# sinhvt3421/scann--material

Measured on AMD Instinct MI355X. Metric: QM9 molecules/s forward, higher is better.
Workload: dtype f32 (projections: split-fp16 hi/lo operands, 3 v_mfma_f32_32x32x16_f16 per product, fp32 accumulate; everything else fp32)

## Files before the change

### scann--material_amd/csrc/scann_forward.cpp

```cpp
#include "scann_runtime.h"

namespace {

constexpr unsigned kTimingEventFlags = hipEventDisableSystemFence;

int ensure_debug(scann_handle* h, scann_dbatch* db) {
  const int L = h->cfg.n_attention;
  if (db->dbg_layers == L) return SCANN_OK;
  HIPCHK(h, cached_malloc((void**)&db->dbg_c, (size_t)(L + 1) * db->n_atom * D * 4));
  HIPCHK(h, cached_malloc((void**)&db->dbg_ctx, (size_t)std::max(L, 1) * db->n_atom * D * 4));
  if (h->cfg.g_update) HIPCHK(h, cached_malloc((void**)&db->dbg_g, (size_t)(L + 1) * std::max(db->n_edge, 1) * D * 4));
  db->dbg_layers = L;
  return SCANN_OK;
}

int ensure_outputs(scann_handle* h, scann_dbatch* db, const FwdOpts& o) {
  db->out_layers = o.train ? 0 : o.out_layers;
  db->out_flags = o.train ? 0 : o.out_flags;
  db->out_attn = db->out_z = db->out_bf = nullptr;
  if (!db->out_layers && !db->out_flags) return SCANN_OK;
  const scann_config_t& c = h->cfg;
  const size_t n_attn = (size_t)__builtin_popcountll(db->out_layers) * db->n_edge * c.num_head;
  const size_t n_z = db->out_flags & SCANN_OUT_AFTER_LC ? (size_t)db->n_atom * c.global_dim : 0;
  const size_t n_bf = db->out_flags & SCANN_OUT_BF_PROPERTY ? (size_t)db->n_struct * c.dense_out : 0;
// ... 182 lines not shown
  bool on;
  std::vector<hipEvent_t> ev;
  std::vector<int> kind;
  void mark(int k) {
    if (!on) return;
    hipEvent_t e;
    (void)hipEventCreateWithFlags(&e, kTimingEventFlags);
    (void)hipEventRecord(e, s);
    ev.push_back(e);
    kind.push_back(k);
  }
};

int run_forward(scann_handle* h, scann_dbatch* db, hipStream_t s, const FwdOpts& o) {
  scann_handle* const W = o.n_member ? o.members[0] : o.weights ? o.weights : h;
  const FwdTrain* const tr = o.train;
  const McState* const mc = o.mc;
  Timer* const tm = o.tm;
  const bool debug = o.keep_layers < 0 ? h->debug : o.keep_layers != 0;
  const bool exact = o.exact || ((h->force_exact || W->weights_exact) && !debug && !tr);
  const int nm = o.n_member;
  const int64_t wst = o.m_w, ast = o.m_a;
  if (!o.of_set) {
    db->idle = false;
    db->fwd_pending = true;
  }
  if (!W->loaded) return fail(h, SCANN_ERR_WEIGHTS, "forward: weights not loaded");
  const scann_config_t& c = h->cfg;
  const int L = c.n_attention;
  const bool outs = o.out_flags != FWD_OUT_UNTOUCHED;
  const bool fuse_basis = !exact && (h->fuse_basis || mc) && c.g_update && L > 0 && !debug && !tr && db->n_edge > 0;
  if (outs && !tr && o.out_layers && !h->generic && c.g_update && !exact && !fuse_basis && db->n_edge > 0)
    return fail(h, SCANN_ERR_UNSUPPORTED, "forward: local-attention outputs need the fused first layer (not with scann_set_debug or SCANN_FUSE_BASIS=0)");
  HIPCHK(h, wait_upload(db, s));
  if (outs)
    if (const int r = ensure_outputs(h, db, o)) return r;
  const FwdBufs b = o.bufs ? *o.bufs : FwdBufs(db);
  if (h->generic) {
    if (tm) { tm->mark(-1); }
    const int r = run_forward_generic(h, db, s, o, W, b);
    if (tm) tm->mark(3);
    return r;
  }
  if (debug) {
    const int r = ensure_debug(h, db);
    if (r) return r;
  }
  const size_t nA_ = (size_t)db->n_atom * D, nE_ = (size_t)db->n_edge * D;
  auto c_of = [&](int l) { return debug ? db->dbg_c + (size_t)l * nA_ : b.c; };
  auto ctx_of = [&](int l) { return debug ? db->dbg_ctx + (size_t)l * nA_ : b.ctx; };
  auto g_of = [&](int l) { return debug && c.g_update ? db->dbg_g + (size_t)l * nE_ : b.geom; };
  int32_t* const rflag = h->range_flag ? h->range_flag + (o.slot >= 0 ? o.slot : db->last_slot) : nullptr;
  if (tm) tm->mark(-1);
  if (!fuse_basis) {
    if (c.g_update) launch_basis(W->basis, db->dist, db->weight, db->n_edge, g_of(0), s);
    else launch_basis_raw(W->cd, db->dist, db->n_edge, b.gd, s);
  }
  if (tm) tm->mark(0);

  const bool general_embed = c.use_ring || c.feature_cgcnn;
  if (general_embed) {
    for (int m = 0; m < std::max(nm, 1); ++m) {
      EmbedArgs e = nm ? o.members[m]->embed : W->embed;
      e.n_atom = db->n_atom; e.atomic = db->atomic;
      e.c0 = reinterpret_cast<float*>(reinterpret_cast<char*>(b.c0) + m * ast);
      e.ring = c.use_ring ? db->ring : nullptr;
      e.cgcnn = c.feature_cgcnn ? db->cgcnn : nullptr;
      launch_embed(e, s);
    }
    if (tm) tm->mark(0);
  }
  const bool species0 = fuse_basis && h->species_tables && !general_embed && !(mc && mc->p_drop > 0.f) && W->sp_c && db->n_big == 0;
  bool sp_dirty = W->sp_dirty;
  for (int m = 1; m < nm; ++m) sp_dirty |= o.members[m]->sp_dirty;
  if (species0 && sp_dirty) {
    AtomArgs a{};
    a.n_atom = c.n_atoms; a.x = W->lut; a.ffn = 0; a.c = W->sp_c;
    a.range_flag = rflag; a.layer = 0;
    const LayerParams& p = W->layers[0];
    a.mode = 0;
    a.WAh = p.W1h; a.bA = p.bg; a.WBh = p.W3h; a.WCh = p.Wqh; a.bC = p.bq;
    a.oA = W->sp_P1; a.oB = W->sp_P3; a.oC = W->sp_q;
    a.n_member = nm; a.m_w = a.m_x = a.m_o = wst;
    launch_atom(a, s);
    HIPCHK(h, hipStreamSynchronize(s));
    W->sp_dirty = false;
    for (int m = 1; m < nm; ++m) o.members[m]->sp_dirty = false;
  }
  const bool keep_bwd = tr && tr->keep_backward;
  for (int l = 0; l <= L; ++l) {
    const bool keep = keep_bwd && db->keep_K && l < L;
    AtomArgs a{};
    a.n_atom = db->n_atom;
    a.n_member = nm; a.m_w = wst; a.m_x = a.m_o = ast;
    if (l == 0) {
      a.x = general_embed ? b.c0 : W->lut;
      a.x_index = general_embed ? nullptr : db->atomic;
      a.ffn = 0;
      if (!general_embed) a.m_x = wst;
    } else {
      a.x = ctx_of(l - 1);
      a.x_index = nullptr;
      a.ffn = c.use_attn_norm ? 1 : 0;
      const LayerParams& pp = W->layers[l - 1];
      a.Wf1h = pp.Wf1h; a.bf1 = pp.bf1; a.Wf2h = pp.Wf2h; a.bf2 = pp.bf2; a.lnr_g = pp.lnr_g; a.lnr_b = pp.lnr_b;
      if (a.ffn && keep_bwd && db->keep_T2) {
        a.keep_pre1 = db->keep_pre1 + (size_t)(l - 1) * nA_; a.keep_H1 = db->keep_H1 + (size_t)(l - 1) * nA_;
        a.keep_T2 = db->keep_T2 + (size_t)(l - 1) * nA_;
      }
    }
    a.c = c_of(l);
    a.range_flag = rflag; a.layer = l;
    if (tr && tr->drop_p > 0.f) {
      a.drop_p = (l == 0 || c.use_attn_norm) ? tr->drop_p : 0.f;
      a.drop_seed = tr->seed;
      a.drop_tag = l == 0 ? DROP_TAG_EMBED : (unsigned)(l - 1);
    }
    if (mc && mc->p_drop > 0.f && (l == 0 || c.use_attn_norm)) {
      a.drop_p = mc->p_drop;
      a.drop_seed = mc->seed;
      a.drop_tag = l == 0 ? DROP_TAG_EMBED : (unsigned)(l - 1);
      a.mc_rows = mc->rows;
      a.mc_t = mc->t;
    }
    if (l < L) {
      const LayerParams& p = W->layers[l];
      a.mode = c.g_update ? 0 : 1;
      a.WAh = p.W1h; a.bA = p.bg; a.WBh = p.W3h; a.WCh = p.Wqh; a.bC = p.bq;
      a.oA = b.P1; a.oB = b.P3; a.oC = keep ? db->keep_q + (size_t)l * nA_ : b.q;
    } else {
      a.mode = 2;
      a.WAh = W->head.Wah; a.bA = W->head.ba; a.WCh = W->head.Wgqh; a.bC = W->head.bgq; a.WDh = W->head.Wgkh; a.bD = W->head.bgk;
      a.oB = b.gk; a.oC = b.gq;
      if (keep_bwd && db->keep_preA) { a.keep_preA = db->keep_preA; a.keep_z = db->keep_z; }
      a.out_z = outs ? db->out_z : nullptr;
    }
#ifdef SCANN_STAMPS
    if (getenv("SCANN_STAMP_ATOM") && l >= 1 && l < L) {
      const int nt = (db->n_atom + 31) / 32;
      if (!db->stamps) HIPCHK(h, hipMalloc((void**)&db->stamps, (size_t)nt * 16 * sizeof(unsigned long long)));
      a.stamps = db->stamps;
      db->n_stamp = nt;
    }
#endif
    if (exact) {
      a.exact = 1;
      if (l > 0 && a.ffn) {
        const LayerParams& pp = W->layers[l - 1];
        a.Wf1h = reinterpret_cast<const _Float16*>(pp.Wf1p); a.Wf2h = reinterpret_cast<const _Float16*>(pp.Wf2p);
      }
      if (l < L) {
        const LayerParams& p = W->layers[l];
        a.WAh = reinterpret_cast<const _Float16*>(p.W1p); a.WBh = reinterpret_cast<const _Float16*>(p.W3p);
        a.WCh = reinterpret_cast<const _Float16*>(p.Wqp);
      } else {
        a.WAh = reinterpret_cast<const _Float16*>(W->head.Wap); a.WCh = reinterpret_cast<const _Float16*>(W->head.Wgqp);
        a.WDh = reinterpret_cast<const _Float16*>(W->head.Wgkp);
      }
    }
    if (!(species0 && l == 0)) launch_atom(a, s);
    if (tm) tm->mark(l < L ? 1 : 3);
    if (l == L) break;
    EdgeArgs ea{};
    ea.tiles = db->tiles; ea.n_tile = db->n_tile; ea.g_update = c.g_update; ea.tile_rows = db->tile_rows;
    ea.edge_offset = db->edge_offset; ea.edge_col = db->edge_col; ea.edge_row = db->edge_row;
    ea.geom = g_of(l); ea.geom_out = debug && c.g_update ? g_of(l + 1) : nullptr; ea.gd = b.gd; ea.edge_weight = db->weight;
    if (fuse_basis && l == 0) { ea.fuse_basis = 1; ea.dist = db->dist; ea.basis = W->basis; }
    ea.n_edge = db->n_edge;
    ea.geom_rows = fuse_basis ? 0 : 1;
    ea.geom_dead = (l == L - 1 && !debug) ? 1 : 0;
    ea.c = c_of(l); ea.P1 = b.P1; ea.P3 = b.P3; ea.q = keep ? db->keep_q + (size_t)l * nA_ : b.q; ea.ctx = ctx_of(l);
    ea.n_member = nm; ea.m_w = wst; ea.m_a = ea.m_r = ast;
    if (species0 && l == 0) { ea.species = db->atomic; ea.c = W->sp_c; ea.P1 = W->sp_P1; ea.P3 = W->sp_P3; ea.q = W->sp_q; ea.m_r = wst; }
    if (keep) {
      ea.keep_V = db->keep_V + (size_t)l * nE_; ea.keep_K = db->keep_K + (size_t)l * nE_;
      if (db->keep_T) ea.keep_T = db->keep_T + (size_t)l * nE_;
      if (db->keep_ang) ea.keep_ang = db->keep_ang + (size_t)l * nE_;
      db->kept = true;
    }
    ea.p = W->layers[l];
    if (exact) {
      ea.exact = 1;
      ea.p.W2h = reinterpret_cast<const _Float16*>(ea.p.W2p); ea.p.Wkh = reinterpret_cast<const _Float16*>(ea.p.Wkp);
    }
    ea.range_flag = rflag; ea.layer = l;
    const bool sample = !tm && !mc && !o.of_set && h->time_every > 0 && (h->time_count % h->time_every) == 0 && !(fuse_basis && l == 0) &&
                        !(ea.geom_dead && L > 2);
    hipEvent_t ev0 = nullptr, ev1 = nullptr;
    if (sample) {
      (void)hipEventCreateWithFlags(&ev0, kTimingEventFlags);
      (void)hipEventCreateWithFlags(&ev1, kTimingEventFlags);
      (void)hipEventRecord(ev0, s);
    }
    ea.tile_part = db->tile_part; ea.part_buf = b.part_buf;
    ea.xcd_remap = h->xcd_remap;
    ea.attn_out = outs ? attn_out_of(h, db, l) : nullptr;
    if (tr && tr->attn_p > 0.f) {
      ea.attn_drop_p = tr->attn_p;
      ea.attn_drop_seed = tr->seed;
      ea.attn_drop_tag = DROP_TAG_ATTN + (unsigned)l;
    }
    if (mc && mc->p_attn > 0.f && db->n_edge > 0) {
      ea.attn_drop_p = mc->p_attn;
      ea.attn_drop_seed = mc->seed;
      ea.attn_drop_tag = DROP_TAG_ATTN + (unsigned)l;
      ea.mc_rows = mc->rows;
      ea.mc_t = mc->t;
    }
#ifdef SCANN_STAMPS
    if (!getenv("SCANN_STAMP_ATOM") && l == (getenv("SCANN_STAMP_LAYER") ? atoi(getenv("SCANN_STAMP_LAYER")) : L - 1)) {
      if (!db->stamps) HIPCHK(h, hipMalloc((void**)&db->stamps, (size_t)db->n_tile * 16 * sizeof(unsigned long long)));
      ea.stamps = db->stamps;
      db->n_stamp = db->n_tile;
    }
#endif
    launch_edge(ea, s);
    if (nm) launch_edge_merge_set(db->big_tab, db->n_big, b.part_buf, ea.q, ea.p.ln_g, ea.p.ln_b, ea.ctx, rflag, l, nm, ast, wst, s);
    else launch_edge_merge(db->big_tab, db->n_big, b.part_buf, ea.q, ea.p.ln_g, ea.p.ln_b, ea.ctx, rflag, l, s);
    if (ea.attn_out) launch_attn_merge(db->big_tab, db->n_big, b.part_buf, db->edge_offset, db->tile_rows, ea.attn_out, s);
    if (sample) {
      (void)hipEventRecord(ev1, s);
      h->time_ev.push_back(ev0);
      h->time_ev.push_back(ev1);
      h->time_edges.push_back(db->n_edge);
    }
    if (tm) tm->mark(2);
  }
  if (!tm && !mc && !o.of_set) h->time_count++;
  ReadoutArgs r{};
  r.mol_offset = db->mol_offset; r.n_struct = db->n_struct; r.max_atoms = db->max_atoms;
  r.gq = b.gq; r.gk = b.gk; r.use_ga_norm = c.use_ga_norm; r.relu_out = W->cfg.relu_out;
  for (int m = 1; m < nm; ++m) r.relu_out |= o.members[m]->cfg.relu_out << m;
  r.p = W->head; r.ga_attn = b.ga; r.y = b.y; r.bf_out = outs ? db->out_bf : nullptr;
  r.n_member = nm; r.m_w = wst; r.m_a = ast; r.m_g = o.m_g; r.m_y = o.m_y;
  launch_readout(r, s);
  if (tm) tm->mark(3);
  HIPCHK(h, hipGetLastError());
  return SCANN_OK;
}

}

extern "C" {
// ... 226 lines not shown
```

### scann--material_amd/csrc/scann_internal.h

```cpp
#pragma once
#include <hip/hip_runtime.h>
#include <stdint.h>

#include <string>
#include <vector>

namespace scann {

constexpr int D = 128;
constexpr int NHEAD = 8;
constexpr int HDIM = D / NHEAD;
constexpr int NG = 20;
constexpr int LDS_STRIDE = 132;
constexpr int TE_MAX = 64;
constexpr int TA = 64;
constexpr int TQ = 24;
constexpr int WPACK = D * D;
constexpr float WSCALE = 256.f;
constexpr float WMAX = 65504.f / WSCALE;

__host__ __device__ inline float drop_scale(unsigned long long seed, unsigned tag, size_t idx, float p) {
  unsigned long long z = seed + 0x9E3779B97F4A7C15ull * (idx + 1) + ((unsigned long long)tag << 48);
  z = (z ^ (z >> 30)) * 0xBF58476D1CE4E5B9ull;
  z = (z ^ (z >> 27)) * 0x94D049BB133111EBull;
// ... 62 lines not shown
struct EdgeTile {
  int32_t atom_begin, atom_end;
  int32_t edge_begin, edge_end;
};

struct LayerParams {
  const float *bg;
  const float *bq;
  const _Float16 *W1h, *W3h, *Wqh, *Wf1h, *Wf2h;
  const float *bk;
  const _Float16 *W2h, *Wkh;
  const _Float16 *Wfh;
  const float *lng_g, *lng_b;
  const float *ln_g, *ln_b;
  const float *Wfg, *bfg;
  const float *bf1, *bf2, *lnr_g, *lnr_b;
  const float *W1p, *W2p, *W3p, *Wqp, *Wkp, *Wf1p, *Wf2p;
};

struct HeadParams {
  const float *Wap, *ba;
  const float *Wgqp, *bgq, *Wgkp, *bgk;
  const _Float16 *Wah, *Wgqh, *Wgkh;
  const float *Wb, *bb;
  const float *wo, *bo;
};

struct BasisParams {
  const float *Wd, *bd, *Ww, *bw;
  const float *cd, *cw;
  const _Float16 *Wdh, *Wwh;
};


void launch_embed_lut(const float* emb, const float* W, const float* b, int n_species, int emb_dim,
                      float* lut, hipStream_t s);

void launch_basis(const BasisParams& p, const float* dist, const float* weight, int n_edge,
                  float* geom, hipStream_t s);
void launch_basis_raw(const float* cd, const float* dist, int n_edge, float* gd, hipStream_t s);

struct EmbedArgs {
  int32_t n_atom, emb_dim;
  const int32_t* atomic;
  const float* cgcnn;
  const float* ring;
  const float *emb;
  const float *We, *be;
  const float *Wr, *br;
  const float *Wde, *bde;
  float* c0;
};
void launch_embed(const EmbedArgs& a, hipStream_t s);

struct AtomArgs {
  const float* x;
  const int32_t* x_index;
  int32_t n_atom;
  int32_t ffn;
  const _Float16 *Wf1h, *Wf2h;
  const float *bf1, *bf2, *lnr_g, *lnr_b;
  float* c;
  float drop_p;
  uint32_t drop_tag;
  unsigned long long drop_seed;
  int32_t mode;
  const _Float16 *WAh, *WBh, *WCh, *WDh;
  const float *bA;
  const float *bC;
  const float *bD;
  float *oA, *oB, *oC;
  float *keep_pre1, *keep_H1, *keep_T2;
  float *keep_preA, *keep_z;
  unsigned long long* stamps;
  int32_t* range_flag;
  int32_t layer;
  int32_t exact;
  float* out_z;
  const McRow* mc_rows;
  uint32_t mc_t;
  int32_t n_member;
  int64_t m_w, m_x, m_o;
};
void launch_atom(const AtomArgs& a, hipStream_t s);

struct EdgeArgs {
  const EdgeTile* tiles;
  int32_t n_tile;
  int32_t xcd_remap;
  const int32_t* tile_part;
  float* part_buf;
  int32_t g_update;
  const int32_t* edge_offset;
  const int32_t* edge_col;
  const int32_t* edge_row;
  float* geom;
  float *keep_V, *keep_T, *keep_ang, *keep_K;
  float* geom_out;
  int32_t tile_rows;
  int32_t n_edge;
  int32_t geom_rows;
  int32_t geom_dead;
  const float* gd;
  const float* edge_weight;
  int32_t fuse_basis;
  const int32_t* species;
  const float* dist;
  BasisParams basis;
  const float *c, *P1, *P3, *q;
  float* ctx;
  float attn_drop_p;
  uint32_t attn_drop_tag;
  unsigned long long attn_drop_seed;
  unsigned long long* stamps;
  int32_t* range_flag;
  int32_t layer;
  int32_t exact;
  LayerParams p;
  float* attn_out;
  const McRow* mc_rows;
  uint32_t mc_t;
  int32_t n_member;
  int64_t m_w, m_r, m_a;
};
void launch_edge(const EdgeArgs& a, hipStream_t s);
void launch_attn_merge(const int32_t* big_tab, int n_big, const float* part_buf, const int32_t* edge_offset, int chunk, float* attn, hipStream_t s);
void launch_edge_merge(const int32_t* big_tab, int n_big, const float* part_buf, const float* q, const float* ln_g,
                       const float* ln_b, float* ctx, int32_t* range_flag, int layer, hipStream_t s);
void launch_edge_merge_set(const int32_t* big_tab, int n_big, const float* part_buf, const float* q, const float* ln_g, const float* ln_b,
                           float* ctx, int32_t* range_flag, int layer, int n_member, int64_t m_a, int64_t m_w, hipStream_t s);

struct GenSeg {
  const float* p;
  const int32_t* idx;
  int32_t w;
};
struct GenDenseArgs {
  GenSeg seg[3];
  int32_t n_seg;
  int32_t prod;
  const float* W;
  const float* b;
  int32_t K, N, rows;
  int32_t act;
  const float* res;
  const int32_t* res_idx;
  const float* row_scale;
  float* Y;
  float* pre;
  float drop_p;
  uint32_t drop_tag;
  unsigned long long drop_seed;
  const McRow* mc_rows;
  uint32_t mc_t;
};
void launch_gen_dense(const GenDenseArgs& a, hipStream_t s);
void launch_gen_layernorm(const float* X, const float* res, const float* gamma, const float* beta, int rows, int N, float* Y, hipStream_t s);
void launch_gen_gauss(const float* x, const float* centres, int n, float* out, hipStream_t s);
void launch_gen_mul(const float* a, const float* b, size_t n, float* out, hipStream_t s);
void launch_gen_attn(const float* q, const float* K, const int32_t* edge_offset, int n_atom, int d, int H, int max_degree, float* ctx, hipStream_t s,
                     float drop_p = 0.f, unsigned drop_tag = 0, unsigned long long drop_seed = 0, float* attn_out = nullptr);
void launch_gen_attn_mc(const float* q, const float* K, const int32_t* edge_offset, int n_atom, int d, int H, int max_degree, float* ctx, hipStream_t s,
                        float drop_p, unsigned drop_tag, unsigned long long drop_seed, const McRow* mc_rows, uint32_t mc_t);
void launch_mc_rows(const int32_t* mol_offset, const int32_t* edge_offset, const unsigned long long* keys, int n_struct, int n_atom, McRow* rows,
                    hipStream_t s);
void launch_mc_reduce(const float* samples, int T, int n, float* mean, float* std_out, hipStream_t s);
void launch_gen_readout(const int32_t* mol_offset, int n_struct, int max_atoms, const float* gq, const float* gk, int dg, int dout, int use_ga_norm,
// ... 129 lines not shown
```

### scann--material_amd/csrc/scann_kernels.hip

```cpp
#include <algorithm>
#include <cstdlib>
#include <type_traits>
#include "scann_internal.h"
#include "scann_mma.h"

namespace scann {


__device__ __forceinline__ void mc_row_key(const AtomArgs& a, int atom, unsigned long long& seed, size_t& e) {
  const McRow m = a.mc_rows[atom];
  seed = mc_seed(a.drop_seed, a.mc_t, m.key);
  e = (size_t)(atom - m.a0) * D;
}
__device__ __forceinline__ float4 mc_drop4(unsigned long long seed, unsigned tag, size_t e, float p, float4 v) {
  v.x *= drop_scale(seed, tag, e, p);
  v.y *= drop_scale(seed, tag, e + 1, p);
  v.z *= drop_scale(seed, tag, e + 2, p);
  v.w *= drop_scale(seed, tag, e + 3, p);
  return v;
}
__device__ __forceinline__ float4 mc_keep4(uint32_t bits, float p, float4 v) {
  const float sc = 1.0f / (1.0f - p);
  v.x *= (bits & 1u) ? sc : 0.f;
  v.y *= (bits & 2u) ? sc : 0.f;
  v.z *= (bits & 4u) ? sc : 0.f;
  v.w *= (bits & 8u) ? sc : 0.f;
  return v;
}
template <class T>
__device__ __forceinline__ T* set_member(T* p, int64_t bytes) {
  return reinterpret_cast<T*>(reinterpret_cast<typename std::conditional<std::is_const<T>::value, const char, char>::type*>(p) + bytes);
}
template <bool FFN, int MODE, int RT, bool EX = false, bool KEEP = false, bool ZOUT = false, bool MC = false, bool SET = false>
__global__ __launch_bounds__(256, RT == 2 ? (EX ? 2 : 3) : (MODE == 1 ? 3 : 4)) void atom_kernel(AtomArgs a) {
#pragma clang fp contract(off)
  static_assert(!(EX && KEEP), "the training forward runs the split-fp16 kernels");
  static_assert(!ZOUT || (MODE == 2 && !KEEP), "after_Lc is an output of the readout launch of inference forwards");
  static_assert(!MC || (!EX && !KEEP && !ZOUT), "Monte Carlo dropout runs on the plain split-fp16 inference kernels");
  static_assert(!SET || (!EX && !KEEP && !ZOUT && !MC), "a model set runs the plain split-fp16 inference kernels");
  constexpr int TAR = 32 * RT;
  unsigned set_bix = blockIdx.x;
  if constexpr (SET) {
    const unsigned nt = ((unsigned)a.n_atom + TAR - 1) / TAR, m = blockIdx.x / nt;
    set_bix = blockIdx.x - m * nt;
    const int64_t w = (int64_t)m * a.m_w, o = (int64_t)m * a.m_o;
    a.x = set_member(a.x, (int64_t)m * a.m_x);
    a.Wf1h = set_member(a.Wf1h, w); a.Wf2h = set_member(a.Wf2h, w);
    a.bf1 = set_member(a.bf1, w); a.bf2 = set_member(a.bf2, w); a.lnr_g = set_member(a.lnr_g, w); a.lnr_b = set_member(a.lnr_b, w);
    a.WAh = set_member(a.WAh, w); a.WBh = set_member(a.WBh, w); a.WCh = set_member(a.WCh, w); a.WDh = set_member(a.WDh, w);
    a.bA = set_member(a.bA, w); a.bC = set_member(a.bC, w); a.bD = set_member(a.bD, w);
    a.c = set_member(a.c, o); a.oA = set_member(a.oA, o); a.oB = set_member(a.oB, o); a.oC = set_member(a.oC, o);
  }
  __shared__ __attribute__((aligned(16))) unsigned char sTile[2 * TAR * PLANE_STRIDE * 2];
  __shared__ __attribute__((aligned(16))) float sRed[TAR * 8];
#ifdef SCANN_DIAG_SE_ROWMAJOR
#define SR_STAT(w, r) (((r) * 4 + (w)) * 2)
#else
#define SR_STAT(w, r) (((w) * TAR + (r)) * 2)
#endif
  __shared__ __attribute__((aligned(16))) float sPar[7 * D];
#define SCANN_ATOM_BIX set_bix
#include "scann_atom_body.inc"
#undef SR_STAT
#undef SCANN_ATOM_BIX
}

void launch_atom(const AtomArgs& a, hipStream_t s) {
  if (a.n_atom <= 0) return;
  const int rows = a.n_atom <= 32 * 1024 ? 32 : 64;
  if (a.n_member > 0) {
    const dim3 grid(((a.n_atom + rows - 1) / rows) * a.n_member), block(256);
#define SCANN_ATOM_SET(F, M)                                                                                          \
  do {                                                                                                                \
    if (rows == 32) hipLaunchKernelGGL((atom_kernel<F, M, 1, false, false, false, false, true>), grid, block, 0, s, a); \
    else hipLaunchKernelGGL((atom_kernel<F, M, 2, false, false, false, false, true>), grid, block, 0, s, a);           \
  } while (0)
    if (a.ffn) {
      if (a.mode == 0) SCANN_ATOM_SET(true, 0);
      else if (a.mode == 1) SCANN_ATOM_SET(true, 1);
      else SCANN_ATOM_SET(true, 2);
    } else {
      if (a.mode == 0) SCANN_ATOM_SET(false, 0);
      else if (a.mode == 1) SCANN_ATOM_SET(false, 1);
      else SCANN_ATOM_SET(false, 2);
    }
#undef SCANN_ATOM_SET
    return;
  }
  const dim3 grid((a.n_atom + rows - 1) / rows), block(256);
  if (a.mc_rows && a.drop_p > 0.f) {
#define SCANN_ATOM_MC(F, M)                                                                                   \
  do {                                                                                                        \
    if (rows == 32) hipLaunchKernelGGL((atom_kernel<F, M, 1, false, false, false, true>), grid, block, 0, s, a); \
    else hipLaunchKernelGGL((atom_kernel<F, M, 2, false, false, false, true>), grid, block, 0, s, a);           \
  } while (0)
    if (a.ffn) {
      if (a.mode == 0) SCANN_ATOM_MC(true, 0);
      else if (a.mode == 1) SCANN_ATOM_MC(true, 1);
      else SCANN_ATOM_MC(true, 2);
    } else {
      if (a.mode == 0) SCANN_ATOM_MC(false, 0);
      else if (a.mode == 1) SCANN_ATOM_MC(false, 1);
      else SCANN_ATOM_MC(false, 2);
    }
#undef SCANN_ATOM_MC
    return;
  }
  const bool keep = !a.exact && (a.drop_p > 0.f || a.keep_pre1 || a.keep_T2 || a.keep_preA);
  if (a.mode == 2 && a.out_z) {
#define SCANN_ATOM_Z(F)                                                                                        \
  do {                                                                                                         \
    if (a.exact) {                                                                                             \
      if (rows == 32) hipLaunchKernelGGL((atom_kernel<F, 2, 1, true, false, true>), grid, block, 0, s, a);     \
      else hipLaunchKernelGGL((atom_kernel<F, 2, 2, true, false, true>), grid, block, 0, s, a);                \
    } else if (rows == 32) hipLaunchKernelGGL((atom_kernel<F, 2, 1, false, false, true>), grid, block, 0, s, a); \
    else hipLaunchKernelGGL((atom_kernel<F, 2, 2, false, false, true>), grid, block, 0, s, a);                 \
  } while (0)
    if (a.ffn) SCANN_ATOM_Z(true);
    else SCANN_ATOM_Z(false);
#undef SCANN_ATOM_Z
    return;
  }
#define SCANN_ATOM_CASE(F, M)                                                                               \
  do {                                                                                                      \
    if (a.exact) {                                                                                          \
      if (rows == 32) hipLaunchKernelGGL((atom_kernel<F, M, 1, true>), grid, block, 0, s, a);               \
      else hipLaunchKernelGGL((atom_kernel<F, M, 2, true>), grid, block, 0, s, a);                          \
    } else if (keep) {                                                                                      \
      if (rows == 32) hipLaunchKernelGGL((atom_kernel<F, M, 1, false, true>), grid, block, 0, s, a);        \
      else hipLaunchKernelGGL((atom_kernel<F, M, 2, false, true>), grid, block, 0, s, a);                   \
    } else if (rows == 32) hipLaunchKernelGGL((atom_kernel<F, M, 1>), grid, block, 0, s, a);                \
    else hipLaunchKernelGGL((atom_kernel<F, M, 2>), grid, block, 0, s, a);                                  \
  } while (0)
  if (a.ffn) {
    if (a.mode == 0) SCANN_ATOM_CASE(true, 0);
    else if (a.mode == 1) SCANN_ATOM_CASE(true, 1);
    else SCANN_ATOM_CASE(true, 2);
  } else {
    if (a.mode == 0) SCANN_ATOM_CASE(false, 0);
    else if (a.mode == 1) SCANN_ATOM_CASE(false, 1);
    else SCANN_ATOM_CASE(false, 2);
  }
#undef SCANN_ATOM_CASE
}


template <bool GUPD, int RT, bool FB = false, bool EX = false, bool KEEP = false, bool DEAD = false, bool ATTN = false, bool MC = false,
          bool SET = false>
__global__ __launch_bounds__(256, RT == 2 ? 3 : 4) void edge_kernel(EdgeArgs a) {
#pragma clang fp contract(off)
  static_assert(!FB || GUPD, "the fused basis exists for the g_update kernel only");
  static_assert(!(FB && EX), "the exact fallback runs the plain first layer");
  static_assert(!KEEP || (!FB && !EX && !DEAD), "the training forward runs the plain split-fp16 kernel and keeps every layer's geometry");
  static_assert(!DEAD || GUPD, "the base branch stores no geometry");
  static_assert(!(ATTN && KEEP), "the training forward returns no attention weights");
  static_assert(!MC || (!EX && !KEEP && !ATTN), "Monte Carlo dropout runs on the split-fp16 inference kernels and returns no attention weights");
  static_assert(!SET || (!EX && !KEEP && !ATTN && !MC), "a model set runs the split-fp16 inference kernels and returns no attention weights");
  constexpr int TEK = 32 * RT;
  constexpr bool BLK = GUPD && !EX && !KEEP;
  __shared__ __attribute__((aligned(16))) unsigned char sTile[2 * TEK * PLANE_STRIDE * 2];
  __shared__ __attribute__((aligned(16))) float sQ[TQ * LDS_STRIDE];
  __shared__ __attribute__((aligned(16))) float sE[NHEAD * (TEK + 1)];
#ifdef SCANN_DIAG_SE_ROWMAJOR
#define SE_STAT(w, r) (((r) * 4 + (w)) * 2)
#define SE_LOGIT(r, h) ((r) * NHEAD + (h))
#else
#define SE_STAT(w, r) (((w) * TEK + (r)) * 2)
#define SE_LOGIT(r, h) ((h) * (TEK + 1) + (r))
#endif
  __shared__ __attribute__((aligned(16))) float sPar[5 * D];
  __shared__ int sOff[TQ + 1];
#ifdef SCANN_DIAG_OCC2
  __shared__ float sDummy[7 * 1024];
  if (a.n_tile < 0) sDummy[threadIdx.x] = 1.f;
#endif
  static_assert(2 * TEK * PLANE_STRIDE * 2 >= TEK * LDS_STRIDE * (int)sizeof(float), "K tile must fit the plane buffer");
  int set_tix = 0;
  if constexpr (SET) {
    const int t = a.xcd_remap ? xcd_tile(blockIdx.x, gridDim.x) : blockIdx.x, m = t / a.n_tile;
    set_tix = t - m * a.n_tile;
    const int64_t w = (int64_t)m * a.m_w, r = (int64_t)m * a.m_r, x = (int64_t)m * a.m_a;
    a.p.W2h = set_member(a.p.W2h, w); a.p.Wkh = set_member(a.p.Wkh, w); a.p.Wfh = set_member(a.p.Wfh, w);
    a.p.bfg = set_member(a.p.bfg, w); a.p.bk = set_member(a.p.bk, w);
    a.p.lng_g = set_member(a.p.lng_g, w); a.p.lng_b = set_member(a.p.lng_b, w); a.p.ln_g = set_member(a.p.ln_g, w); a.p.ln_b = set_member(a.p.ln_b, w);
    a.basis.Wdh = set_member(a.basis.Wdh, w); a.basis.Wwh = set_member(a.basis.Wwh, w); a.basis.bd = set_member(a.basis.bd, w);
    a.basis.bw = set_member(a.basis.bw, w); a.basis.cd = set_member(a.basis.cd, w); a.basis.cw = set_member(a.basis.cw, w);
    a.c = set_member(a.c, r); a.P1 = set_member(a.P1, r); a.P3 = set_member(a.P3, r); a.q = set_member(a.q, r);
    a.geom = set_member(a.geom, x); a.ctx = set_member(a.ctx, x); a.part_buf = set_member(a.part_buf, x);
  }
#define SCANN_EDGE_TIX (SET ? set_tix : a.xcd_remap ? xcd_tile(blockIdx.x, gridDim.x) : blockIdx.x)
#include "scann_edge_body.inc"
// ... 477 lines not shown
```

### scann--material_amd/csrc/scann_runtime.cpp

```cpp
#include "scann_runtime.h"

#include <mutex>

namespace {

struct BlockCache {
  std::multimap<size_t, void*> free_blocks;
  std::map<void*, size_t> size_of;
  size_t cached_bytes = 0;
};
std::map<int, BlockCache> g_block_cache;
std::mutex g_block_mu;
constexpr size_t BLOCK_CACHE_LIMIT = (size_t)16 << 30;
thread_local std::string g_create_error;

std::vector<WeightSpec> build_specs(const scann_config_t& c) {
  std::vector<WeightSpec> s;
  const int64_t d = c.local_dim, dg = c.global_dim, dout = c.dense_out, emb = c.embedding_dim;
  if (c.feature_cgcnn) {
    s.push_back({"embed_atom/kernel", 92, emb});
    s.push_back({"embed_atom/bias", emb, 0});
  } else {
    s.push_back({"embed_atom/embeddings", c.n_atoms, emb});
  }
// ... 158 lines not shown
    shift += -14 - e;
    base = 0;
  } else {
    base = (uint32_t)(e + 15) << 10;
    m &= 0x7FFFFFu;
  }
  const uint32_t q = m >> shift, rem = m & ((1u << shift) - 1), halfway = 1u << (shift - 1);
  uint32_t r = base + q;
  if (rem > halfway || (rem == halfway && (q & 1))) ++r;
  return (uint16_t)(sign | r);
}
static float f16_bits_to_f32(uint16_t h) {
  const uint32_t sign = (uint32_t)(h & 0x8000u) << 16, e = (h >> 10) & 31, m = h & 0x3FFu;
  float out;
  if (e == 0) {
    out = std::ldexp((float)m, -24);
  } else if (e == 31) {
    uint32_t x = 0x7F800000u | (m << 13);
    memcpy(&out, &x, 4);
  } else {
    out = std::ldexp((float)(m | 0x400u), (int)e - 25);
  }
  uint32_t x;
  memcpy(&x, &out, 4);
  x |= sign;
  memcpy(&out, &x, 4);
  return out;
}
void pack_weight_f16(const float* W, int ld, int k_real, int ks, uint16_t* out) {
  for (int w = 0; w < 4; ++w)
    for (int s = 0; s < ks; ++s)
      for (int lane = 0; lane < 64; ++lane)
        for (int j = 0; j < 8; ++j) {
          const int k = 16 * s + 8 * (lane >> 5) + j;
          const float x = k < k_real ? WSCALE * W[(size_t)k * ld + 32 * w + (lane & 31)] : 0.f;
          const uint16_t hi = f32_to_f16_bits(x);
          const uint16_t lo = f32_to_f16_bits(x - f16_bits_to_f32(hi));
          const size_t base = ((size_t)(w * ks + s) * 2) * 64 * 8 + (size_t)lane * 8 + j;
          out[base] = hi;
          out[base + 64 * 8] = lo;
        }
}

}

extern "C" {

int scann_abi_version(void) { return SCANN_ABI_VERSION; }

int scann_device_count(void) {
  int n = 0;
  if (hipGetDeviceCount(&n) != hipSuccess) return 0;
  return n;
}

const char* scann_last_error(const scann_handle_t* h) { return h ? h->err.c_str() : g_create_error.c_str(); }

int scann_create(const scann_config_t* cfg, int device_id, scann_handle_t** out) {
  if (!cfg || !out) return fail(nullptr, SCANN_ERR_INVALID, "scann_create: null argument");
  *out = nullptr;
  if (cfg->n_gauss != NG) return fail(nullptr, SCANN_ERR_UNSUPPORTED, "scann_create: 20 Gaussians (custom_layers.py:39-53 as called by scann_model.py:378,384)");
  const bool generic = cfg->local_dim != D || cfg->global_dim != D || cfg->dense_out != D || cfg->num_head != NHEAD ||
                       (getenv("SCANN_GENERIC") && atoi(getenv("SCANN_GENERIC")));
  if (generic) {
    if (cfg->local_dim <= 0 || cfg->num_head <= 0 || cfg->global_dim <= 0 || cfg->dense_out <= 0 || cfg->local_dim % cfg->num_head != 0)
      return fail(nullptr, SCANN_ERR_INVALID, "scann_create: local_dim must be a positive multiple of num_head (attention.py:170-173), global_dim and dense_out positive");
    if (cfg->local_dim > 1024 || cfg->global_dim > 1024 || cfg->dense_out > 1024 || cfg->embedding_dim > 1024)
      return fail(nullptr, SCANN_ERR_UNSUPPORTED, "scann_create: widths above 1024 are not implemented");
  } else if (cfg->embedding_dim + (cfg->use_ring ? 10 : 0) > 160) {
    return fail(nullptr, SCANN_ERR_UNSUPPORTED, "scann_create: embedding_dim (+10 ring features) must be <= 160");
  }
  if (cfg->n_atoms <= 0 || cfg->embedding_dim <= 0 || cfg->n_attention < 0 || !(cfg->gaussian_d > 0))
    return fail(nullptr, SCANN_ERR_INVALID, "scann_create: bad hyper-parameter");
  int ndev = 0;
  if (hipGetDeviceCount(&ndev) != hipSuccess || ndev <= 0)
    return fail(nullptr, SCANN_ERR_NO_DEVICE, "scann_create: no HIP device visible (this library has no CPU fallback)");
  if (device_id < 0 || device_id >= ndev) return fail(nullptr, SCANN_ERR_NO_DEVICE, "scann_create: device_id out of range");
  scann_handle* h = new scann_handle();
  h->cfg = *cfg;
  h->generic = generic;
  h->device = device_id;
  h->specs = build_specs(*cfg);
  if (const char* xr = getenv("SCANN_XCD_REMAP")) h->xcd_remap = atoi(xr) != 0;
  if (const char* fb = getenv("SCANN_FUSE_BASIS")) h->fuse_basis = atoi(fb) != 0;
  if (const char* st = getenv("SCANN_SPECIES_TABLES")) h->species_tables = atoi(st) != 0;
  if (const char* sg = getenv("SCANN_STRICT_RANGE")) h->strict_range = atoi(sg) != 0;
  if (const char* fe = getenv("SCANN_EXACT")) h->force_exact = atoi(fe) != 0;
  {
    hipDeviceProp_t prop;
    if (hipGetDeviceProperties(&prop, device_id) == hipSuccess && prop.multiProcessorCount > 0) h->n_cu = prop.multiProcessorCount;
  }
  if (const char* ns = getenv("SCANN_STREAMS")) h->nstream = std::min(MAX_STREAM, std::max(1, atoi(ns)));
  if (hipSetDevice(device_id) != hipSuccess) {
    delete h;
    return fail(nullptr, SCANN_ERR_HIP, "scann_create: hipSetDevice failed");
  }
  if (hipHostMalloc((void**)&h->range_flag, 128, hipHostMallocDefault) != hipSuccess) {
    delete h;
    return fail(nullptr, SCANN_ERR_HIP, "scann_create: hipHostMalloc failed");
  }
  for (int i = 0; i < 32; ++i) h->range_flag[i] = 0;
  for (int i = 0; i < h->nstream; ++i) {
    if (hipStreamCreateWithFlags(&h->streams[i], hipStreamNonBlocking) != hipSuccess) {
      delete h;
      return fail(nullptr, SCANN_ERR_HIP, "scann_create: hipStreamCreate failed");
    }
  }
  *out = h;
  return SCANN_OK;
}

void scann_destroy(scann_handle_t* h) {
  if (!h) return;
  (void)hipSetDevice(h->device);
  (void)hipDeviceSynchronize();
  for (int i = 0; i < MAX_STREAM; ++i)
    if (h->streams[i]) (void)hipStreamDestroy(h->streams[i]);
  if (h->d_weights) (void)hipFree(h->d_weights);
  for (scann_handle::DlStage& st : h->dl_stage)
    if (st.p) (void)hipHostFree(st.p);
  if (h->g_weights) (void)hipFree(h->g_weights);
  if (h->g_centres) (void)hipFree(h->g_centres);
  if (h->g_WT) (void)hipFree(h->g_WT);
  if (h->d_gt_descs) (void)hipFree(h->d_gt_descs);
  if (h->sp_c) (void)hipFree(h->sp_c);
  for (scann_handle::Stage& st : h->stage) {
    if (st.p) (void)hipHostFree(st.p);
    if (st.ev) (void)hipEventDestroy(st.ev);
  }
  if (h->copy_stream) (void)hipStreamDestroy(h->copy_stream);
  for (void* q : {(void*)h->t_master, (void*)h->t_grad, (void*)h->t_m, (void*)h->t_v, (void*)h->t_l2, (void*)h->t_descs, (void*)h->ig_grad})
    if (q) (void)hipFree(q);
  if (h->comm) ncclCommDestroy(h->comm);
  if (h->train_aux && !h->train_aux_borrowed) (void)hipStreamDestroy(h->train_aux);
  if (h->h_stat) (void)hipHostFree(h->h_stat);
  if (h->range_flag) (void)hipHostFree(h->range_flag);
  for (float* t : h->h_targets)
    if (t) (void)hipHostFree(t);
  for (hipEvent_t e : h->step_ev)
    if (e) (void)hipEventDestroy(e);
  if (h->train_aux2) (void)hipStreamDestroy(h->train_aux2);
  for (hipEvent_t e : h->train_ev) (void)hipEventDestroy(e);
  for (hipEvent_t e : h->time_ev) (void)hipEventDestroy(e);
  free_models(h->models);
  if (h->sc_db) free_batch(h->sc_db);
  if (h->sc_arena) (void)hipFree(h->sc_arena);
  if (h->pp_dev) (void)hipFree(h->pp_dev);
  if (h->pp_host) (void)hipHostFree(h->pp_host);
  if (h->sc_host) (void)hipHostFree(h->sc_host);
  cache_release(h->device);
  delete h;
}

int scann_num_streams(const scann_handle_t* h) { return h ? h->nstream : 0; }

int scann_weight_count(const scann_handle_t* h) { return h ? (int)h->specs.size() : SCANN_ERR_INVALID; }

int scann_weight_name(const scann_handle_t* h, int index, const char** name, int64_t* rows, int64_t* cols) {
  if (!h || index < 0 || index >= (int)h->specs.size()) return SCANN_ERR_INVALID;
  if (name) *name = h->specs[index].name.c_str();
  if (rows) *rows = h->specs[index].rows;
  if (cols) *cols = h->specs[index].cols;
  return SCANN_OK;
}

int64_t scann_param_count(const scann_handle_t* h) {
// ... 328 lines not shown
```

### scann--material_amd/csrc/scann_runtime.h

```cpp
#pragma once
#include "../../include/scann_hip.h"
#include "scann_internal.h"
#include "scann_train.h"

#include <rccl/rccl.h>

#include <algorithm>
#include <cmath>
#include <cstdlib>
#include <cstring>
#include <map>
#include <memory>
#include <string>
#include <vector>

using namespace scann;

namespace scann {

constexpr int MAX_STREAM = 16;

hipError_t cached_malloc(void** p, size_t bytes);
void cached_free(void* p);
void cache_release(int dev);
// ... 6 lines not shown

struct GenLayerKeep {
  float *cc_in = nullptr, *G_in = nullptr;
  float *Z = nullptr;
  float *T = nullptr;
  float *Gn = nullptr;
  float *K = nullptr, *q = nullptr;
  float *t1 = nullptr, *ctx = nullptr;
  float *pre1 = nullptr, *h1 = nullptr, *t2 = nullptr;
  float *cc_out = nullptr;
};
struct GenKeep {
  char* arena = nullptr;
  size_t bytes = 0;
  char* barena = nullptr;
  size_t bbytes = 0;
  std::vector<GenLayerKeep> layer;
  float *embE = nullptr, *ring10 = nullptr, *pre_e = nullptr, *cc0 = nullptr;
  float *gd = nullptr, *gw = nullptr, *pre_d = nullptr, *pre_w = nullptr, *Td = nullptr, *Tw = nullptr, *G0 = nullptr;
  float *cc_L = nullptr, *z_pre = nullptr, *z = nullptr, *gq = nullptr, *gk = nullptr, *rep = nullptr, *hid_pre = nullptr, *hid = nullptr;
  float drop_p = 0.f, attn_p = 0.f;
  unsigned long long seed = 0;
  std::map<std::string, std::pair<const float*, size_t>> dbg;
};

struct scann_train_ws {
  char* arena = nullptr;
  std::vector<float*> tA;
  float *keep_q = nullptr, *keep_V = nullptr, *keep_T = nullptr, *keep_ang = nullptr, *keep_K = nullptr;
  float *keep_pre1 = nullptr, *keep_H1 = nullptr, *keep_T2 = nullptr;
  float *keep_preA = nullptr, *keep_z = nullptr;
  std::vector<float*> tE;
  float *rep = nullptr, *dpre = nullptr, *dy = nullptr, *targets = nullptr, *dlut = nullptr;
  float* wpart = nullptr;
  size_t wpart_floats = 0;
  float* det_part = nullptr;
  size_t det_floats = 0;
  double* sse = nullptr;
  char* ig = nullptr;
  size_t ig_bytes = 0;
  float drop_p = 0.f, attn_p = 0.f;
  unsigned long long seed = 0;
  GenKeep gen;
  ~scann_train_ws() {
    cached_free(arena);
    cached_free(det_part);
    cached_free(ig);
    cached_free(gen.arena);
    cached_free(gen.barena);
  }
};

struct Timer;
struct ModelSet;
void free_models(ModelSet* ms);

struct McState {
  const McRow* rows;
  unsigned long long seed;
  uint32_t t;
  float p_drop, p_attn;
};

}

struct scann_handle {
  scann_config_t cfg{};
  int device = 0;
  std::string err;
  hipStream_t streams[MAX_STREAM]{};
  int nstream = 2;
  std::vector<WeightSpec> specs;
  bool loaded = false;
  bool debug = false;
  uint64_t out_layers = 0;
  int32_t out_flags = 0;
  int tile_atoms = TQ;
  int n_cu = 256;
  int time_every = 0;
  int64_t time_count = 0;
  std::vector<hipEvent_t> time_ev;
  std::vector<int> time_edges;
  int xcd_remap = 1;
  int fuse_basis = 1;
  int species_tables = 1;
  bool generic = false;
  float* g_weights = nullptr;
  float* g_centres = nullptr;
  std::map<std::string, int64_t> g_off;
  std::vector<GenTransDesc> gt_descs;
  GenTransDesc* d_gt_descs = nullptr;
  std::map<std::string, int64_t> gt_off;
  float* g_WT = nullptr;
  int gt_max = 0;
  bool weights_exact = false;
  bool force_exact = false;
  bool strict_range = false;
  int64_t exact_reruns = 0;
  float* d_weights = nullptr;
  std::vector<LayerParams> layers;
  HeadParams head{};
  BasisParams basis{};
  const float* lut = nullptr;
  float *sp_c = nullptr, *sp_P1 = nullptr, *sp_P3 = nullptr, *sp_q = nullptr;
  bool sp_dirty = true;
  const float* cd = nullptr;
  EmbedArgs embed{};
  std::vector<float> host_master;
  std::vector<int64_t> spec_off;
  std::vector<RepackDesc> descs;
  size_t arena_floats = 0, o_lut = 0, o_emb = 0, o_Wde = 0, o_bde = 0;
  struct LayerT {
    const float *W1T, *W2T, *W3T, *WqT, *WkT, *Wf1T, *Wf2T;
    const _Float16 *W1Th, *W2Th, *W3Th, *WqTh, *WkTh, *Wf1Th, *Wf2Th;
  };
  std::vector<LayerT> layersT;
  const float *WaT = nullptr, *WgqT = nullptr, *WgkT = nullptr;
  const _Float16* WaTh = nullptr;
  float *t_master = nullptr, *t_grad = nullptr, *t_m = nullptr, *t_v = nullptr, *t_l2 = nullptr;
  RepackDesc* t_descs = nullptr;
  float* ig_grad = nullptr;
  int64_t t_step = 0;
  float attn_drop_p = 0.f;
  bool deterministic = false;
  ncclComm_t comm = nullptr;
  double* h_stat = nullptr;
  float* h_targets[3] = {nullptr, nullptr, nullptr};
  size_t h_targets_cap[3] = {0, 0, 0};
  hipEvent_t step_ev[2] = {nullptr, nullptr};
  int64_t step_begun = 0, step_ended = 0;
  bool grads_zeroed = false;
  struct Stage { char* p = nullptr; size_t cap = 0; hipEvent_t ev = nullptr; bool used = false; };
  static constexpr int N_STAGE = 8;
  Stage stage[N_STAGE];
  int stage_next = 0;
  struct PadScratch { std::vector<int32_t> gidx, at, mol, eoff, col; std::vector<float> dist, wgt, ga; };
  PadScratch pad_scratch;
  struct DlStage { char* p = nullptr; size_t cap = 0; };
  DlStage dl_stage[MAX_STREAM];
  hipStream_t copy_stream = nullptr;
  hipStream_t train_aux2 = nullptr;
  bool train_fused = true;
  bool train_aux_borrowed = false;
  hipStream_t train_aux = nullptr;
  std::vector<hipEvent_t> train_ev;
  char* sc_arena = nullptr;
  size_t sc_cap = 0;
  char* pp_host = nullptr;
  char* pp_dev = nullptr;
  size_t pp_cap = 0;
  char* sc_host = nullptr;
  size_t sc_host_cap = 0;
  struct scann_dbatch* sc_db = nullptr;
  int comm_world = 1;
  int32_t* range_flag = nullptr;
  ModelSet* models = nullptr;
  uint64_t models_gen = 0;
};

struct scann_dbatch {
  int32_t n_struct = 0, n_atom = 0, n_edge = 0, n_tile = 0, max_atoms = 0, tile_rows = 64, max_degree = 0, tile_atoms = TQ;
  char* arena = nullptr;
  int32_t *atomic = nullptr, *mol_offset = nullptr, *edge_offset = nullptr, *edge_col = nullptr, *edge_row = nullptr;
  float *dist = nullptr, *weight = nullptr, *ring = nullptr, *cgcnn = nullptr, *c0 = nullptr;
  EdgeTile* tiles = nullptr;
  float *keep_q = nullptr, *keep_V = nullptr, *keep_T = nullptr, *keep_ang = nullptr, *keep_K = nullptr;
// ... 119 lines not shown
```

Measured before the change: 2.018 million.

## Add 96-row wide atom tiles and occupancy-aware tile-row selection

Adds a 96-row atom kernel variant for plain inference ResidualNorm launches (FFN, mode 0/2). It also picks the atom tile height from the atom count relative to CU count, so the grid fills the device while per-block weight loads are amortised over more rows. An env override SCANN_ATOM_ROWS is added. The larger tile uses more LDS and fewer blocks, which may lower occupancy or leave the tail unbalanced. It also changes the default 32/64 choice for the eligible path.

```diff
diff --git a/scann--material_amd/csrc/scann_forward.cpp b/scann--material_amd/csrc/scann_forward.cpp
--- a/scann--material_amd/csrc/scann_forward.cpp
+++ b/scann--material_amd/csrc/scann_forward.cpp
@@ -288,7 +288,7 @@
     a.WAh = p.W1h; a.bA = p.bg; a.WBh = p.W3h; a.WCh = p.Wqh; a.bC = p.bq;
     a.oA = W->sp_P1; a.oB = W->sp_P3; a.oC = W->sp_q;
     a.n_member = nm; a.m_w = a.m_x = a.m_o = wst;
-    launch_atom(a, s);
+    launch_atom(a, s, h->n_cu, h->atom_rows);
     HIPCHK(h, hipStreamSynchronize(s));
     W->sp_dirty = false;
     for (int m = 1; m < nm; ++m) o.members[m]->sp_dirty = false;
@@ -364,7 +364,7 @@
         a.WDh = reinterpret_cast<const _Float16*>(W->head.Wgkp);
       }
     }
-    if (!(species0 && l == 0)) launch_atom(a, s);
+    if (!(species0 && l == 0)) launch_atom(a, s, h->n_cu, h->atom_rows);
     if (tm) tm->mark(l < L ? 1 : 3);
     if (l == L) break;
     EdgeArgs ea{};
diff --git a/scann--material_amd/csrc/scann_internal.h b/scann--material_amd/csrc/scann_internal.h
--- a/scann--material_amd/csrc/scann_internal.h
+++ b/scann--material_amd/csrc/scann_internal.h
@@ -168,7 +168,7 @@
   int32_t n_member;
   int64_t m_w, m_x, m_o;
 };
-void launch_atom(const AtomArgs& a, hipStream_t s);
+void launch_atom(const AtomArgs& a, hipStream_t s, int n_cu, int force_rows);
 
 struct EdgeArgs {
   const EdgeTile* tiles;
diff --git a/scann--material_amd/csrc/scann_kernels.hip b/scann--material_amd/csrc/scann_kernels.hip
--- a/scann--material_amd/csrc/scann_kernels.hip
+++ b/scann--material_amd/csrc/scann_kernels.hip
@@ -65,9 +65,44 @@
 #undef SCANN_ATOM_BIX
 }
 
-void launch_atom(const AtomArgs& a, hipStream_t s) {
+template <bool FFN, int MODE, int RT>
+__global__ __launch_bounds__(256, 2) void atom_wide_kernel(AtomArgs a) {
+#pragma clang fp contract(off)
+  static_assert(FFN && (MODE == 0 || MODE == 2) && RT == 3, "the wide tiles exist for the ResidualNorm launches of plain inference forwards");
+  constexpr bool EX = false, KEEP = false, ZOUT = false, MC = false;
+  constexpr int TAR = 32 * RT;
+  __shared__ __attribute__((aligned(16))) unsigned char sTile[2 * TAR * PLANE_STRIDE * 2];
+  __shared__ __attribute__((aligned(16))) float sRed[TAR * 8];
+#define SR_STAT(w, r) (((w) * TAR + (r)) * 2)
+  __shared__ __attribute__((aligned(16))) float sPar[7 * D];
+#define SCANN_ATOM_BIX blockIdx.x
+#include "scann_atom_body.inc"
+#undef SR_STAT
+#undef SCANN_ATOM_BIX
+}
+
+static int atom_tile_rows(const AtomArgs& a, int n_cu, bool wide, int force) {
+  if (force == 32 || force == 64 || (wide && force == 96)) return force;
+  const int rows = a.n_atom <= 32 * 1024 ? 32 : 64;
+  if (!wide || n_cu <= 0) return rows;
+  if ((a.n_atom + 31) / 32 <= 3 * n_cu) return 32;
+  if ((a.n_atom + 63) / 64 <= 2 * n_cu) return 64;
+  if ((a.n_atom + 95) / 96 <= 2 * n_cu) return 96;
+  return 64;
+}
+
+void launch_atom(const AtomArgs& a, hipStream_t s, int n_cu, int force_rows) {
   if (a.n_atom <= 0) return;
-  const int rows = a.n_atom <= 32 * 1024 ? 32 : 64;
+  const bool keep = !a.exact && (a.drop_p > 0.f || a.keep_pre1 || a.keep_T2 || a.keep_preA);
+  const bool wide = a.ffn && (a.mode == 0 || a.mode == 2) && !a.exact && !keep && a.n_member <= 0 && !(a.mc_rows && a.drop_p > 0.f) &&
+                    !(a.mode == 2 && a.out_z);
+  const int rows = atom_tile_rows(a, n_cu, wide, force_rows);
+  if (rows == 96) {
+    const dim3 grid((a.n_atom + rows - 1) / rows), block(256);
+    if (a.mode == 0) hipLaunchKernelGGL((atom_wide_kernel<true, 0, 3>), grid, block, 0, s, a);
+    else hipLaunchKernelGGL((atom_wide_kernel<true, 2, 3>), grid, block, 0, s, a);
+    return;
+  }
   if (a.n_member > 0) {
     const dim3 grid(((a.n_atom + rows - 1) / rows) * a.n_member), block(256);
 #define SCANN_ATOM_SET(F, M)                                                                                          \
@@ -106,7 +141,6 @@
 #undef SCANN_ATOM_MC
     return;
   }
-  const bool keep = !a.exact && (a.drop_p > 0.f || a.keep_pre1 || a.keep_T2 || a.keep_preA);
   if (a.mode == 2 && a.out_z) {
 #define SCANN_ATOM_Z(F)                                                                                        \
   do {                                                                                                         \
diff --git a/scann--material_amd/csrc/scann_runtime.cpp b/scann--material_amd/csrc/scann_runtime.cpp
--- a/scann--material_amd/csrc/scann_runtime.cpp
+++ b/scann--material_amd/csrc/scann_runtime.cpp
@@ -264,6 +264,7 @@
   h->device = device_id;
   h->specs = build_specs(*cfg);
   if (const char* xr = getenv("SCANN_XCD_REMAP")) h->xcd_remap = atoi(xr) != 0;
+  if (const char* ar = getenv("SCANN_ATOM_ROWS")) h->atom_rows = atoi(ar);
   if (const char* fb = getenv("SCANN_FUSE_BASIS")) h->fuse_basis = atoi(fb) != 0;
   if (const char* st = getenv("SCANN_SPECIES_TABLES")) h->species_tables = atoi(st) != 0;
   if (const char* sg = getenv("SCANN_STRICT_RANGE")) h->strict_range = atoi(sg) != 0;
diff --git a/scann--material_amd/csrc/scann_runtime.h b/scann--material_amd/csrc/scann_runtime.h
--- a/scann--material_amd/csrc/scann_runtime.h
+++ b/scann--material_amd/csrc/scann_runtime.h
@@ -112,6 +112,7 @@
   std::vector<hipEvent_t> time_ev;
   std::vector<int> time_edges;
   int xcd_remap = 1;
+  int atom_rows = 0;
   int fuse_basis = 1;
   int species_tables = 1;
   bool generic = false;
```

Result: faster. 2.058 million (median of 6 runs) (+2.0%).
